# IwakuraRein/CIS-565-Final-VR-Raytracer

Measured on AMD Instinct MI355X. Metric: Mrays/s (ClosestHit+AnyHit ray queries per second) of the 1080p ReSTIR DI+GI+denoise frame; ms_per_step = ms/frame, higher is better.
Workload: dtype f32

## Files before the change

### cis-565-final-vr-raytracer_amd/csrc/dev_scene.h

```cpp
#pragma once
#include <hip/hip_runtime.h>
#include "bvh8.h"
#include "../../include/rt_abi.h"

namespace rt {

struct DevInstance {
  float o2w[12];
  float w2o[12];
  uint32_t primMesh;
  uint32_t flags;
  uint32_t pad[2];
};

struct DevTexture {
  const uint8_t* bgra;
  int32_t w, h, wrapS, wrapT, filter, pad;
};

struct DevScene {
  const Node8* nodes;
  const Tri48* tris;
  const TriRef* triRef;
  const AlphaRec* alphaRec;
  const AlphaRec* alphaByTri;
  const DevInstance* instances;
  const rt_prim_mesh* primMeshes;
  const rt_vertex* vertices;
  const uint32_t* indices;
  const rt_material* materials;
  const DevTexture* textures;
  const rt_punc_light* puncLights;
  const rt_trig_light* trigLights;
  const float* env;
  const rt_impt_samp* envAccel;
  rt_light_buf_info lightInfo;
  int32_t envW, envH;
  uint32_t numTris, numNodes;
  const struct SkyPre* sky;
  int32_t stackEntries;
  int32_t coopLive;
  float triPad;
  int32_t stackTotal;
  uint2* stackOvf; uint2* stackOvfInd;
  uint32_t stackOvfThreads;
  int32_t gangMax;
};

struct SurfRec {
  rt_vec3 position, normal, ffnormal, emission;
  float roughness, metallic;
  uint32_t matID, seed;
};

struct DevFrame {
  uint4* thisG; const uint4* lastG;
  short2* motion;
  rt_direct_reservoir* thisDirectResv; const rt_direct_reservoir* lastDirectResv;
  rt_indirect_reservoir* thisIndirectResv; const rt_indirect_reservoir* lastIndirectResv;
  uint32_t* thisLightId; const uint32_t* lastLightId;
  float4* thisDirectResult; float4* thisIndirectResult;
  float4* denoiseDirA; float4* denoiseDirB; float4* denoiseIndA; float4* denoiseIndB;
  unsigned long long* counters;
  SurfRec* surf; uint32_t* status; uint32_t* qcount; uint32_t* waveProf;
  float4* geomN; float4* geomP; float4* geomNh; float4* geomPh;
  rt_direct_reservoir* tempDirectResv;
  double* postRowSums; float* postMean;
  float4* postMipD; float4* postMipI;
  uint32_t* tileOrder;
  int32_t W, H;
  int32_t histRow0, histRow1;
  uint32_t* histMiss;
  int32_t stackLds;
  int32_t pad4;
  const uint32_t* seedIn; uint32_t* seedOut;
};

struct OmCamera {
  rt_mat4 lastProjView;
  rt_vec3 lastPosition; float pad;
};
struct DevObjMotion {
  uint32_t* instImage;
  const OmCamera* cams;
  uint32_t numInst, pad;
};

}
```

### cis-565-final-vr-raytracer_amd/csrc/rt_api.cpp

```cpp
#include <hip/hip_runtime.h>
#include <array>
#include <atomic>
#include <memory>
#include <mutex>
#include <cmath>
#include <cstdio>
#include <map>
#include <cstdlib>
#include <chrono>
#include <cstring>
#include <string>
#include <thread>
#include <unordered_map>
#include <vector>
#include "../../include/rt_abi.h"
#include "../../include/rt_cpus.h"
#include "bvh8_builder.h"
#include "stages.h"
#include "reference.h"
#include "svgf.h"
#include "gi_spatial.h"
#include "taa.h"
#include "refit.h"
#include "accel_build.h"
// ... 663 lines not shown
    if(!alphaOf.empty() && alphaOf[T.globalId]) { T.alphaIdx = alphaOf[T.globalId]; memcpy(T.omm, ommOf[T.alphaIdx].data(), sizeof(T.omm)); continue; }
    const TriRef ref = bo.triRef[T.globalId];
    const rt_prim_mesh& pm = c->primMeshes[c->instances[ref.inst].primMesh];
    const rt_material& m = c->materials[size_t(pm.materialIndex > 0 ? pm.materialIndex : 0)];
    const uint32_t* ix = &c->indices[pm.firstIndex + 3 * ref.prim];
    AlphaRec a{};
    int32_t tex = -1;
    const rt_vec2 t0 = c->vertices[pm.vertexOffset + ix[0]].texcoord, t1 = c->vertices[pm.vertexOffset + ix[1]].texcoord, t2 = c->vertices[pm.vertexOffset + ix[2]].texcoord;
    a.uv0x = t0.x; a.uv0y = t0.y; a.uv1x = t1.x; a.uv1y = t1.y; a.uv2x = t2.x; a.uv2y = t2.y;
    a.baseAlpha = m.pbrBaseColorFactor.w; a.cutoff = m.alphaCutoff; a.alphaMode = m.alphaMode;
    if(m.pbrBaseColorTexture > -1 && size_t(m.pbrBaseColorTexture) < c->devTextures.size()) {
      const DevTexture& t = c->devTextures[size_t(m.pbrBaseColorTexture)];
      tex = m.pbrBaseColorTexture; a.w = t.w; a.h = t.h; a.wrapS = t.wrapS; a.wrapT = t.wrapT; a.filter = t.filter;
    }
    T.alphaIdx = uint32_t(alpha.size());
    alpha.push_back(a); alphaTex.push_back(tex);
    std::array<uint32_t, 12> key{};
    memcpy(key.data(), &a.uv0x, 8 * sizeof(float));
    key[8] = uint32_t(m.pbrBaseColorTexture); key[9] = uint32_t(a.alphaMode); key[10] = uint32_t(a.wrapS) ^ (uint32_t(a.wrapT) << 16); key[11] = uint32_t(a.filter);
    auto it = ommCache.find(key);
    if(it == ommCache.end()) {
      std::array<uint32_t, 4> o{};
      const std::vector<uint8_t>* al = (tex >= 0 && size_t(tex) < c->hostAlpha.size()) ? &c->hostAlpha[size_t(m.pbrBaseColorTexture)] : nullptr;
      buildOpacityMap(a, al, o.data());
      it = ommCache.emplace(key, o).first;
    }
    memcpy(T.omm, it->second.data(), sizeof(T.omm));
    if(!alphaOf.empty()) { alphaOf[T.globalId] = T.alphaIdx; ommOf.resize(alpha.size()); ommOf[T.alphaIdx] = it->second; }
  }
  lt.lap("alpha records + micro-maps");
  return RT_OK;
}

int rt_build_accel(rt_ctx* c)
{
  if(!c) return RT_ERR_INVALID_ARG;
  if(!c->haveScene) return fail(c, RT_ERR_NO_SCENE, "rt_build_accel: no scene uploaded");
  RT_HIP(c, hipSetDevice(c->device));
  RT_HIP(c, syncAll(c));
  { const int rc = syncHostVertices(c); if(rc) return rc; }
  freePool(c->accelAllocs); freePool(c->rebuildAllocs);
  c->refit = rt_ctx::Refit{};
  c->rebuild = rt_ctx::Rebuild{};
  c->haveAccel = false;
  c->refN = 0;
  c->svgfValid = false;
  c->taaValid = false;
  std::shared_ptr<const HostAccel> ha;
  LoadTimer lt;
  {
    std::lock_guard<std::mutex> one(g_accelMutex);
    uint64_t k0, k1;
    sceneKey(c, k0, k1);
    lt.lap("scene key");
    if(g_accelCache && g_accelCache->key0 == k0 && g_accelCache->key1 == k1) ha = g_accelCache;
    else {
      auto fresh = std::make_shared<HostAccel>();
      fresh->key0 = k0; fresh->key1 = k1;
      const int rc = buildHostAccel(c, *fresh);
      if(rc) return rc;
      ha = fresh; g_accelCache = ha;
    }
  }
  lt.lap("host products (build or cache)");
  const BuildOutput& bo = ha->bo;
  int rc;
  {
    std::vector<AlphaRec> alpha = ha->alpha;
    for(size_t i = 0; i < alpha.size(); i++) if(ha->alphaTex[i] >= 0) alpha[i].bgra = c->devTextures[size_t(ha->alphaTex[i])].bgra;
    if((rc = upload(c, c->accelAllocs, alpha.data(), alpha.size(), &c->ds.alphaRec))) return rc;
    std::vector<AlphaRec> byTri(bo.tris.size(), AlphaRec{});
    for(size_t i = 0; i < bo.tris.size(); i++) if(!(bo.tris[i].flags & TRI_OPAQUE)) byTri[i] = alpha[bo.tris[i].alphaIdx];
    if((rc = upload(c, c->accelAllocs, byTri.data(), byTri.size(), &c->ds.alphaByTri))) return rc;
  }
  if((rc = upload(c, c->accelAllocs, bo.nodes.data(), bo.nodes.size(), &c->ds.nodes))) return rc;
  if((rc = upload(c, c->accelAllocs, bo.tris.data(), bo.tris.size(), &c->ds.tris))) return rc;
  if((rc = upload(c, c->accelAllocs, bo.triRef.data(), bo.triRef.size(), &c->ds.triRef))) return rc;
  if((rc = upload(c, c->accelAllocs, bo.instances.data(), bo.instances.size(), &c->ds.instances))) return rc;
  c->ds.numNodes = uint32_t(bo.nodes.size()); c->ds.numTris = uint32_t(bo.tris.size());
  c->ds.stackTotal = std::max(8, ((bo.maxDepth + 1 + 3) / 4) * 4);
  c->ds.stackEntries = c->ds.stackTotal;
  c->ds.triPad = bo.pad;
  { const char* e = getenv("RESTIR_COOP"); c->ds.coopLive = e ? std::max(0, std::min(64, atoi(e))) : 4; }
  { const char* e = getenv("RESTIR_GANG"); c->ds.gangMax = e ? std::max(0, std::min(7, atoi(e))) : 4; }
  c->numNodes = bo.nodes.size(); c->numTris = bo.triRef.size(); c->maxDepth = bo.maxDepth;
  c->numRefs = bo.tris.size(); c->spatialSplits = size_t(bo.spatialSplits); c->sahNodeSteps = bo.sahNodeSteps; c->sahTriSteps = bo.sahTriSteps;
  RT_HIP(c, hipDeviceSynchronize());
  lt.lap("uploads (tree, alpha records)");
  c->haveAccel = true;
  reopenPriorityDecision(c);
  if((rc = resetSeedPlane(c))) return rc;
  return ensureStackOverflow(c);
}

int rt_resize(rt_ctx* c, int w, int h)
{
  if(!c) return RT_ERR_INVALID_ARG;
  if(w <= 0 || h <= 0 || w > 32767 || h > 32767) return fail(c, RT_ERR_INVALID_ARG, "rt_resize: size must be in 1..32767 (RG16_SINT motion vectors)");
  RT_HIP(c, hipSetDevice(c->device));
  RT_HIP(c, syncAll(c));
  reopenPriorityDecision(c);
  for(void*& p : c->indA) { if(p && p != c->bufs[RT_BUF_DENOISE_IND_A]) (void)hipFree(p); p = nullptr; }
  for(int i = 0; i < RT_BUF_COUNT; i++) { if(c->bufs[i]) (void)hipFree(c->bufs[i]); c->bufs[i] = nullptr; c->bufBytes[i] = 0; }
  for(void** p : {&c->spareG, &c->spareMotion, &c->spareG2, &c->spareMotion2, &c->spareDirRes}) if(*p) { (void)hipFree(*p); *p = nullptr; }
  c->W = c->H = 0;
  for(void* p : {static_cast<void*>(c->refAcc), static_cast<void*>(c->refMean)}) if(p) (void)hipFree(p);
  c->refAcc = nullptr; c->refMean = nullptr; c->refN = 0;
  freeSvgfHistory(c);
  freeGiSpatial(c);
  freeTaaHistory(c);
  freeObjectMotion(c);
  const size_t n = size_t(w) * h, nh = size_t(w / 2) * (h / 2);
  for(int i = 0; i < RT_BUF_COUNT; i++) {
    const size_t bytes = (halfRes(i) ? nh : n) * elemBytes(i);
    const size_t alloc = bytes + (halfRes(i) ? size_t(w / 2) * (RT_PAD_ROWS / 2) : size_t(w) * RT_PAD_ROWS) * elemBytes(i) + 16;
    RT_HIP(c, hipMalloc(&c->bufs[i], alloc));
    RT_HIP(c, hipMemset(c->bufs[i], (i == RT_BUF_LIGHT_ID0 || i == RT_BUF_LIGHT_ID1) ? 0xff : 0, alloc));
    c->bufBytes[i] = bytes; c->bufAlloc[i] = alloc;
    if(i == RT_BUF_DENOISE_IND_A) {
      c->indA[0] = c->bufs[i];
      RT_HIP(c, hipMalloc(&c->indA[1], alloc));
      RT_HIP(c, hipMemset(c->indA[1], 0, alloc));
    }
    if(i == RT_BUF_GBUFFER0 || i == RT_BUF_MOTION) {
      for(void** spare : {(i == RT_BUF_MOTION) ? &c->spareMotion : &c->spareG, (i == RT_BUF_MOTION) ? &c->spareMotion2 : &c->spareG2}) {
        RT_HIP(c, hipMalloc(spare, alloc));
        RT_HIP(c, hipMemset(*spare, 0, alloc));
      }
    }
    if(i == RT_BUF_DIRECT_RESULT0) {
      RT_HIP(c, hipMalloc(&c->spareDirRes, alloc));
      RT_HIP(c, hipMemset(c->spareDirRes, 0, alloc));
    }
  }
  freePool(c->scratchAllocs);
  c->scratch = DevFrame{};
  auto alloc = [&](size_t bytes, void** out) -> int {
    RT_HIP(c, hipMalloc(out, std::max<size_t>(bytes, 256)));
    c->scratchAllocs.push_back(*out);
    RT_HIP(c, hipMemset(*out, 0, std::max<size_t>(bytes, 256)));
    return RT_OK;
  };
  DevFrame& X = c->scratch;
  int rc;
#define RT_SCRATCH(field, count, T) if((rc = alloc(size_t(count) * sizeof(T), reinterpret_cast<void**>(&X.field)))) return rc
  RT_SCRATCH(surf, n, SurfRec); RT_SCRATCH(status, n, uint32_t); RT_SCRATCH(qcount, 256, uint32_t);
  RT_SCRATCH(geomN, n, float4); RT_SCRATCH(geomP, n, float4); RT_SCRATCH(geomNh, nh, float4); RT_SCRATCH(geomPh, nh, float4);
  RT_SCRATCH(postRowSums, size_t(h) * 6, double); RT_SCRATCH(postMean, 8, float);
  RT_SCRATCH(postMipD, n + 64, float4); RT_SCRATCH(postMipI, n + 64, float4);
  RT_SCRATCH(tileOrder, (size_t(w / 2 + 7) / 8) * (size_t(h / 2 + 7) / 8 + 16 * 2) + 64 + 4096, uint32_t);
  RT_SCRATCH(seedOut, n, uint32_t); X.seedIn = X.seedOut;
#if RT_WAVEPROF
  RT_SCRATCH(waveProf, WAVEPROF_RECORDS * 16, uint32_t);
#endif
#undef RT_SCRATCH
  RT_HIP(c, hipDeviceSynchronize());
  c->W = w; c->H = h;
  if((rc = resetSeedPlane(c))) return rc;
  if(c->objMotion != RT_OBJECT_MOTION_OFF && (rc = allocObjectMotion(c))) return rc;
  return ensureStackOverflow(c);
}

static int ensureStackOverflow(rt_ctx* c)
{
  freePool(c->ovfAllocs);
  c->ds.stackOvf = c->ds.stackOvfInd = nullptr; c->ds.stackOvfThreads = 0;
// ... 1681 lines not shown
```

### cis-565-final-vr-raytracer_amd/csrc/traverse.h

```cpp
#pragma once
#include "dev_math.h"
#include "dev_scene.h"
#include "stages.h"

namespace rt {



struct RayHit {
  float t;
  uint32_t gid;
  float u, v;
};

#ifndef RT_WAVEPROF
#define RT_WAVEPROF 0
#endif
struct TravCounters {
  uint32_t nodes, tris, rounds, live;
#if RT_WAVEPROF
  uint32_t rN, rT, rC, cN, cT, cC, aTex, aOmm;
  uint32_t ph[8];
  uint32_t nph[4];
  uint32_t hl[8], he[8];
#endif
};

RT_DEV int floorMod(int i, int p)
{
  if((p & (p - 1)) == 0) return i & (p - 1);
  int m = i % p; if(m < 0) m += p;
  return m;
}
RT_DEV int wrapCoord(int i, int n, int mode)
{
  if(mode == RT_WRAP_CLAMP) return i < 0 ? 0 : (i >= n ? n - 1 : i);
  if(mode == RT_WRAP_MIRROR) {
    const int p = 2 * n;
    const int m = floorMod(i, p);
    return m < n ? m : p - 1 - m;
  }
  return floorMod(i, n);
}
RT_DEV bool wrapIsMask(int w, int h, int wrapS, int wrapT) { return (((w & (w - 1)) | (h & (h - 1))) == 0) && wrapS == RT_WRAP_REPEAT && wrapT == RT_WRAP_REPEAT; }
RT_DEV bool waveNone(bool c) { return __builtin_amdgcn_ballot_w64(c) == 0ull; }
RT_DEV f4 texelBGRA(const DevTexture& t, int x, int y)
{
  uint32_t p = gLoadU32(t.bgra + (size_t(y) * t.w + x) * 4);
  return mk4(unorm8ToFloat((p >> 16) & 0xffu), unorm8ToFloat((p >> 8) & 0xffu), unorm8ToFloat(p & 0xffu), unorm8ToFloat(p >> 24));
}
RT_DEV f4 sampleTexture(const DevScene& S, int id, f2 uv)
{
  const DevTexture t = S.textures[id];
  float fx = uv.x * float(t.w), fy = uv.y * float(t.h);
  const bool masks = waveNone(!wrapIsMask(t.w, t.h, t.wrapS, t.wrapT));
  if(t.filter == RT_FILTER_NEAREST) {
    const int xi = rt_ftoi(rt_floor(fx)), yi = rt_ftoi(rt_floor(fy));
    if(masks) return texelBGRA(t, xi & (t.w - 1), yi & (t.h - 1));
    return texelBGRA(t, wrapCoord(xi, t.w, t.wrapS), wrapCoord(yi, t.h, t.wrapT));
  }
  fx = fx - 0.5f; fy = fy - 0.5f;
  float x0f = rt_floor(fx), y0f = rt_floor(fy);
  float ax = fx - x0f, ay = fy - y0f;
  int x0 = rt_ftoi(x0f), y0 = rt_ftoi(y0f);
  int xa, xb, ya, yb;
  if(masks) { xa = x0 & (t.w - 1); xb = (x0 + 1) & (t.w - 1); ya = y0 & (t.h - 1); yb = (y0 + 1) & (t.h - 1); }
  else {
    xa = wrapCoord(x0, t.w, t.wrapS); xb = wrapCoord(x0 + 1, t.w, t.wrapS);
    ya = wrapCoord(y0, t.h, t.wrapT); yb = wrapCoord(y0 + 1, t.h, t.wrapT);
  }
  f4 top = mix(texelBGRA(t, xa, ya), texelBGRA(t, xb, ya), ax);
  f4 bot = mix(texelBGRA(t, xa, yb), texelBGRA(t, xb, yb), ax);
  return mix(top, bot, ay);
}
RT_DEV f4 envTexel(const DevScene& S, int x, int y)
{
  const float4 p = gLoadF4(S.env + (size_t(y) * S.envW + x) * 4);
  return mk4(p.x, p.y, p.z, p.w);
}
RT_DEV f4 sampleEnv(const DevScene& S, f2 uv)
{
  float fx = uv.x * float(S.envW) - 0.5f, fy = uv.y * float(S.envH) - 0.5f;
  float x0f = rt_floor(fx), y0f = rt_floor(fy);
  float ax = fx - x0f, ay = fy - y0f;
  int x0 = rt_ftoi(x0f), y0 = rt_ftoi(y0f);
  int xa = wrapCoord(x0, S.envW, RT_WRAP_REPEAT), xb = wrapCoord(x0 + 1, S.envW, RT_WRAP_REPEAT);
  int ya = wrapCoord(y0, S.envH, RT_WRAP_CLAMP), yb = wrapCoord(y0 + 1, S.envH, RT_WRAP_CLAMP);
  f4 top = mix(envTexel(S, xa, ya), envTexel(S, xb, ya), ax);
  f4 bot = mix(envTexel(S, xa, yb), envTexel(S, xb, yb), ax);
  return mix(top, bot, ay);
}

RT_DEV uint32_t pcgNext(uint32_t& state)
{
  uint32_t prev = state * 747796405u + 2891336453u;
  uint32_t word = ((prev >> ((prev >> 28u) + 4u)) ^ prev) * 277803737u;
  state = prev;
// ... 77 lines not shown
  if(F.kind == 1) a00 = gLoadU8(F.p00);
  else if(F.kind == 2) { a00 = gLoadU8(F.p00); a10 = gLoadU8(F.p10); a01 = gLoadU8(F.p01); a11 = gLoadU8(F.p11); }
  return alphaFinish(A, F, a00, a10, a01, a11, gid, raySeed);
}

RT_DEV bool intersectTri(const Tri48& T, f3 o, f3 d, float& t, float& u, float& v)
{
  const f3 e1 = mk3(T.e1x, T.e1y, T.e1z), e2 = mk3(T.e2x, T.e2y, T.e2z), v0 = mk3(T.v0x, T.v0y, T.v0z);
  const f3 p = cross(d, e2);
  const float det = dot(e1, p);
  if(T.flags & TRI_NOCULL) { if(det == 0.0f || rt_isnan(det)) return false; }
  else {
    const float sdet = (T.flags & TRI_FLIP) ? -det : det;
    if(!(sdet > 0.0f)) return false;
  }
  const float inv = 1.0f / det;
  const f3 tv = o - v0;
  u = dot(tv, p) * inv;
  if(!(u >= 0.0f && u <= 1.0f)) return false;
  const f3 q = cross(tv, e1);
  v = dot(d, q) * inv;
  if(!(v >= 0.0f && u + v <= 1.0f)) return false;
  t = dot(e2, q) * inv;
  return !rt_isnan(t);
}
RT_DEV float hitPointPad(f3 o, f3 d, float pad, float t)
{
  const float om = fmaxf(fmaxf(rt_abs(o.x), rt_abs(o.y)), rt_abs(o.z)), dm = fmaxf(fmaxf(rt_abs(d.x), rt_abs(d.y)), rt_abs(d.z));
  return pad + (om + t * dm) * 4.76837158203125e-07f;
}
RT_DEV bool hitInsidePaddedBox(const Tri48& T, f3 o, f3 d, float buildPad, float t)
{
  const float pad = hitPointPad(o, d, buildPad, t);
  const f3 e1 = mk3(T.e1x, T.e1y, T.e1z), e2 = mk3(T.e2x, T.e2y, T.e2z), v0 = mk3(T.v0x, T.v0y, T.v0z);
  const f3 h = o + d * t;
  const f3 lo = mk3((v0.x + fminf(fminf(0.0f, e1.x), e2.x)) - pad, (v0.y + fminf(fminf(0.0f, e1.y), e2.y)) - pad, (v0.z + fminf(fminf(0.0f, e1.z), e2.z)) - pad);
  const f3 hi = mk3((v0.x + fmaxf(fmaxf(0.0f, e1.x), e2.x)) + pad, (v0.y + fmaxf(fmaxf(0.0f, e1.y), e2.y)) + pad, (v0.z + fmaxf(fmaxf(0.0f, e1.z), e2.z)) + pad);
  return h.x >= lo.x && h.x <= hi.x && h.y >= lo.y && h.y <= hi.y && h.z >= lo.z && h.z <= hi.z;
}

RT_DEV float cvtByte(uint32_t w, int j) { return float((w >> (8 * j)) & 0xffu); }

struct Trav {
  f3 o, d;
  float idx, idy, idz;
  uint32_t octinv;
  uint2 ngroup;
  uint2 tgroup;
  int sp;
  float tmax;
  uint32_t seed;
  RayHit hit;
  uint32_t rec;
  bool found;
  bool isAny;
};

RT_DEV bool travHasTris(const Trav& T) { return T.tgroup.y != 0u; }
RT_DEV bool travHasNodes(const Trav& T) { return T.ngroup.y > 0x00FFFFFFu || T.sp > 0; }

template <int MODE>
RT_DEV bool travInit(Trav& T, f3 o, f3 d, float tmax, uint32_t raySeed)
{
  const bool ANY = MODE == 2 ? T.isAny : MODE == 1;
  T.o = o; T.d = d; T.tmax = tmax; T.seed = raySeed; T.found = false; T.sp = 0;
  T.hit.t = ANY ? tmax : RT_INFINITY;
  T.hit.gid = 0xffffffffu; T.hit.u = 0.f; T.hit.v = 0.f; T.rec = 0xffffffffu;
  T.ngroup = make_uint2(0u, 0u);
  T.tgroup = make_uint2(0u, 0u);
  if(hasNan(o) || hasNan(d) || !(T.hit.t > 0.0f)) return false;
  const float eps = 1e-20f;
  T.idx = 1.0f / (rt_abs(d.x) > eps ? d.x : (d.x < 0.0f ? -eps : eps));
  T.idy = 1.0f / (rt_abs(d.y) > eps ? d.y : (d.y < 0.0f ? -eps : eps));
  T.idz = 1.0f / (rt_abs(d.z) > eps ? d.z : (d.z < 0.0f ? -eps : eps));
  T.octinv = (((d.x < 0.0f) ? 1u : 0u) | ((d.y < 0.0f) ? 2u : 0u) | ((d.z < 0.0f) ? 4u : 0u)) ^ 7u;
  T.ngroup = make_uint2(0u, 0x80000000u);
  return true;
}

RT_DEV uint2* stackOverflowSlot(const DevScene& S, int sp)
{
  const size_t thread = size_t(blockIdx.x) * blockDim.x + threadIdx.x;
  return S.stackOvf + (thread * size_t(S.stackTotal - S.stackEntries) + size_t(sp - S.stackEntries));
}
RT_DEV uint2 stackPop(const DevScene& S, Trav& T, uint2* stack)
{
  --T.sp;
  if(__builtin_expect(T.sp < S.stackEntries, 1)) return ldsLoadU2(stack + T.sp * 64);
  return gLoadU2(stackOverflowSlot(S, T.sp));
}
RT_DEV void stackPush(const DevScene& S, Trav& T, uint2* stack, uint2 g)
{
  if(__builtin_expect(T.sp < S.stackEntries, 1)) ldsStoreU2(stack + (T.sp++) * 64, g);
  else if(T.sp < S.stackTotal) { gStoreU2(stackOverflowSlot(S, T.sp), g); T.sp++; }
}

struct NodeRegs { uint4 n0, n1, n2, n3, n4; };
RT_DEV uint32_t travNodeSelect(const DevScene& S, Trav& T, uint2* stack)
{
  uint2 ngroup = T.ngroup;
  if(ngroup.y <= 0x00FFFFFFu) ngroup = stackPop(S, T, stack);
  const uint32_t hits = ngroup.y;
  const uint32_t bit = 31u - uint32_t(__clz(int(hits)));
  ngroup.y &= ~(1u << bit);
  if(ngroup.y > 0x00FFFFFFu) stackPush(S, T, stack, ngroup);
  const uint32_t slot = (bit - 24u) ^ T.octinv;
  const uint32_t rel = uint32_t(__popc(hits & ~(0xFFFFFFFFu << slot) & 0xFFu));
  T.ngroup.y = 0u;
  return ngroup.x + rel;
}
RT_DEV NodeRegs nodeLoad(const DevScene& S, uint32_t index)
{
  const uint4* np = reinterpret_cast<const uint4*>(S.nodes + index);
  NodeRegs N; N.n0 = gLoadU4(np); N.n1 = gLoadU4(np + 1); N.n2 = gLoadU4(np + 2); N.n3 = gLoadU4(np + 3); N.n4 = gLoadU4(np + 4);
  return N;
}
RT_DEV void travNodeTest(Trav& T, const NodeRegs& N)
{
  const uint4 n0 = N.n0, n1 = N.n1, n2 = N.n2, n3 = N.n3, n4 = N.n4;
  const bool nx = T.d.x < 0.0f, ny = T.d.y < 0.0f, nz = T.d.z < 0.0f;
  const uint32_t octinv = T.octinv;
  const uint32_t octinv4 = octinv * 0x01010101u;
  const float adjx = rt_u2f((n0.w & 0xffu) << 23) * T.idx;
  const float adjy = rt_u2f(((n0.w >> 8) & 0xffu) << 23) * T.idy;
  const float adjz = rt_u2f(((n0.w >> 16) & 0xffu) << 23) * T.idz;
  const float orgx = (rt_u2f(n0.x) - T.o.x) * T.idx, orgy = (rt_u2f(n0.y) - T.o.y) * T.idy, orgz = (rt_u2f(n0.z) - T.o.z) * T.idz;
  const uint32_t imask = n0.w >> 24;
  uint32_t hitmask = 0;
#pragma unroll
  for(int half = 0; half < 2; half++) {
    const uint32_t meta4 = half ? n1.w : n1.z;
    const uint32_t isInner4 = (meta4 & (meta4 << 1)) & 0x10101010u;
    const uint32_t innerMask4 = (isInner4 >> 4) * 0xffu;
    const uint32_t bitIndex4 = (meta4 ^ (octinv4 & innerMask4)) & 0x1F1F1F1Fu;
    const uint32_t childBits4 = (meta4 >> 5) & 0x07070707u;
    const uint32_t qlx = half ? n2.y : n2.x, qly = half ? n2.w : n2.z, qlz = half ? n3.y : n3.x;
    const uint32_t qhx = half ? n3.w : n3.z, qhy = half ? n4.y : n4.x, qhz = half ? n4.w : n4.z;
    const uint32_t nearx = nx ? qhx : qlx, farx = nx ? qlx : qhx;
    const uint32_t neary = ny ? qhy : qly, fary = ny ? qly : qhy;
    const uint32_t nearz = nz ? qhz : qlz, farz = nz ? qlz : qhz;
#pragma unroll
    for(int j = 0; j < 4; j++) {
      const float tlx = __builtin_fmaf(cvtByte(nearx, j), adjx, orgx), thx = __builtin_fmaf(cvtByte(farx, j), adjx, orgx);
      const float tly = __builtin_fmaf(cvtByte(neary, j), adjy, orgy), thy = __builtin_fmaf(cvtByte(fary, j), adjy, orgy);
      const float tlz = __builtin_fmaf(cvtByte(nearz, j), adjz, orgz), thz = __builtin_fmaf(cvtByte(farz, j), adjz, orgz);
      const float tn = fmaxf(fmaxf(tlx, tly), fmaxf(tlz, 0.0f));
      const float tf = fminf(fminf(thx, thy), fminf(thz, T.hit.t));
      if(tn <= tf) hitmask |= ((childBits4 >> (8 * j)) & 0xffu) << ((bitIndex4 >> (8 * j)) & 0xffu);
    }
  }
  T.ngroup = make_uint2(n1.x, (hitmask & 0xFF000000u) | imask);
  T.tgroup = make_uint2(n1.y, hitmask & 0x00FFFFFFu);
}
RT_DEV void travNode(const DevScene& S, Trav& T, uint2* stack, TravCounters& tc)
{
  const uint32_t index = travNodeSelect(S, T, stack);
  const NodeRegs N = nodeLoad(S, index);
  tc.nodes++;
  travNodeTest(T, N);
}

struct TriRegs { uint4 a, b, c, om; };
RT_DEV TriRegs triLoad(const DevScene& S, uint32_t triIndex)
{
  const uint4* tp = reinterpret_cast<const uint4*>(S.tris + triIndex);
  TriRegs Q; Q.a = gLoadU4(tp); Q.b = gLoadU4(tp + 1); Q.c = gLoadU4(tp + 2); Q.om = gLoadU4(tp + 3);
// ... 27 lines not shown
    (void)tc;
#endif
    if(state == 1u) return 1;
    if(state == 2u) { uint32_t hs = candidateSeed(seed, R.globalId); return !(rnd(hs) > 0.0f) ? 1 : 0; }
    return 2;
  }
  return 1;
}
RT_DEV bool triCandidate(const DevScene& S, uint32_t triIndex, f3 o, f3 d, bool ANY, float tmax, float curT, uint32_t curG, uint32_t seed, float& t, float& u, float& v,
                         uint32_t& gid, TravCounters& tc)
{
  const TriRegs Q = triLoad(S, triIndex);
  uint32_t alphaIdx;
  const int s = triCandidateGeom(S, Q, o, d, ANY, tmax, curT, curG, seed, t, u, v, gid, alphaIdx, tc);
  if(s == 2) return hitTestAlpha(S, alphaIdx, gid, u, v, seed);
  return s == 1;
}

template <int MODE>
RT_DEV void travTri(const DevScene& S, Trav& T, TravCounters& tc)
{
  const bool ANY = MODE == 2 ? T.isAny : MODE == 1;
  const uint32_t bit = 31u - uint32_t(__clz(int(T.tgroup.y)));
  T.tgroup.y &= ~(1u << bit);
  tc.tris++;
  float t, u, v; uint32_t gid;
  if(!triCandidate(S, T.tgroup.x + bit, T.o, T.d, ANY, T.tmax, T.hit.t, T.hit.gid, T.seed, t, u, v, gid, tc)) return;
  T.hit.t = t; T.hit.gid = gid; T.hit.u = u; T.hit.v = v; T.rec = T.tgroup.x + bit;
  T.found = true;
  if(ANY) { T.tgroup.y = 0u; T.ngroup.y = 0u; T.sp = 0; }
}

RT_DEV float laneF(float v, int l) { return rt_u2f(uint32_t(__builtin_amdgcn_readlane(int(rt_f2u(v)), l))); }
RT_DEV uint32_t laneU(uint32_t v, int l) { return uint32_t(__builtin_amdgcn_readlane(int(v), l)); }

template <int MODE>
RT_DEV void travTriCoop(const DevScene& S, Trav& T, unsigned long long triMask, TravCounters& tc)
{
  const int lane = int(threadIdx.x) & 63;
  const unsigned long long present = __ballot(1);
  const int rank = __popcll(present & ((1ull << lane) - 1ull)), np = __popcll(present);
  while(triMask != 0ull) {
    const int l = __builtin_ctzll(triMask);
    triMask &= triMask - 1ull;
    const f3 o = mk3(laneF(T.o.x, l), laneF(T.o.y, l), laneF(T.o.z, l)), d = mk3(laneF(T.d.x, l), laneF(T.d.y, l), laneF(T.d.z, l));
    const uint32_t tbase = laneU(T.tgroup.x, l), seed = laneU(T.seed, l);
    uint32_t tbits = laneU(T.tgroup.y, l);
    const float tmax = laneF(T.tmax, l);
    const bool ANY = MODE == 2 ? (laneU(T.isAny ? 1u : 0u, l) != 0u) : MODE == 1;
    float bt = laneF(T.hit.t, l), bu = 0.0f, bv = 0.0f;
    uint32_t bg = laneU(T.hit.gid, l), br = 0u;
    bool found = false;
    if(lane == l) tc.tris += uint32_t(__popc(tbits));
    while(tbits != 0u && !(ANY && found)) {
      int mine = -1, j = 0;
      while(tbits != 0u && j < np) {
        const int k = 31 - __clz(int(tbits));
        tbits &= ~(1u << k);
        if(rank == j) mine = k;
        j++;
      }
      float t = 0.0f, u = 0.0f, v = 0.0f; uint32_t gid = 0u;
      bool ok = false;
      if(mine >= 0) ok = triCandidate(S, tbase + uint32_t(mine), o, d, ANY, tmax, bt, bg, seed, t, u, v, gid, tc);
      unsigned long long okm = __ballot(ok ? 1 : 0);
      while(okm != 0ull) {
        const int w = __builtin_ctzll(okm);
        okm &= okm - 1ull;
        const float wt = laneF(t, w); const uint32_t wg = laneU(gid, w);
        if(ANY || wt < bt || (wt == bt && wg < bg)) { bt = wt; bg = wg; bu = laneF(u, w); bv = laneF(v, w); br = tbase + laneU(uint32_t(mine), w); found = true; }
        if(ANY) break;
      }
    }
    if(lane == l) {
      T.tgroup.y = 0u;
      if(found) {
        T.hit.t = bt; T.hit.gid = bg; T.hit.u = bu; T.hit.v = bv; T.rec = br; T.found = true;
        if(ANY) { T.ngroup.y = 0u; T.sp = 0; }
      }
    }
  }
}

template <int ANY>
RT_DEV bool travRound(const DevScene& S, Trav& T, bool live, uint2* stack, TravCounters& tc)
{
  tc.rounds++; tc.live += live ? 1u : 0u;
  const bool wantTri = live && travHasTris(T);
  const bool wantNode = live && !wantTri;
  const int nT = __popcll(__ballot(wantTri ? 1 : 0)), nN = __popcll(__ballot(wantNode ? 1 : 0));
  if(nT >= nN) { if(wantTri) travTri<ANY>(S, T, tc); }
  else { if(wantNode) travNode(S, T, stack, tc); }
  return live && (travHasTris(T) || travHasNodes(T));
}

template <int ANY>
RT_DEV bool travRoundMasked(const DevScene& S, Trav& T, bool live, unsigned long long liveMask, uint2* stack, TravCounters& tc)
{
  tc.rounds++; tc.live += live ? 1u : 0u;
  const bool wantTri = live && travHasTris(T);
  const unsigned long long triMask = __ballot(wantTri ? 1 : 0);
  const int nLive = __popcll(liveMask), nT = __popcll(triMask), nN = nLive - nT;
#if RT_WAVEPROF
  const uint64_t c0 = clock64();
#endif
  if(nLive <= S.coopLive) {
    if(nT > 0) travTriCoop<ANY>(S, T, triMask, tc);
    if(live && travHasNodes(T)) travNode(S, T, stack, tc);
  } else if(nT >= nN) { if(wantTri) travTri<ANY>(S, T, tc); }
  else { if(live && !wantTri) travNode(S, T, stack, tc); }
#if RT_WAVEPROF
  {
    const uint32_t dc = uint32_t(clock64() - c0);
    if(nLive <= S.coopLive) { tc.rC++; tc.cC += dc; } else if(nT >= nN) { tc.rT++; tc.cT += dc; } else { tc.rN++; tc.cN += dc; }
    const int ex = nLive <= S.coopLive ? nLive : (nT >= nN ? nT : nN);
    tc.hl[(nLive - 1) >> 3]++; tc.he[(max(ex, 1) - 1) >> 3]++;
  }
#endif
  return live && (travHasTris(T) || travHasNodes(T));
}

template <int ANY>
RT_DEV bool traceRay(const DevScene& S, f3 o, f3 d, float tmax, uint32_t raySeed, uint2* stack, RayHit& hit, TravCounters& tc)
{
  Trav T;
  bool live = travInit<ANY>(T, o, d, tmax, raySeed);
  unsigned long long liveMask = __ballot(live ? 1 : 0);
  while(liveMask != 0ull) {
    live = travRoundMasked<ANY>(S, T, live, liveMask, stack, tc);
    liveMask = __ballot(live ? 1 : 0);
  }
  hit = T.hit;
  return T.found;
}

RT_DEV bool traceRaySeeded(const DevScene& S, f3 o, f3 d, uint32_t raySeed, uint32_t seedTri, uint2* stack, RayHit& hit, uint32_t& rec, TravCounters& tc)
{
  float st = 0.0f, su = 0.0f, sv = 0.0f; uint32_t sg = 0xffffffffu;
  bool seeded = false;
  if(seedTri < S.numTris) {
    tc.tris++;
    seeded = triCandidate(S, seedTri, o, d, false, RT_INFINITY, RT_INFINITY, 0xffffffffu, raySeed, st, su, sv, sg, tc);
  }
  Trav T;
  bool live = travInit<0>(T, o, d, RT_INFINITY, raySeed);
  if(live && seeded) { T.hit.t = st; T.hit.gid = sg; T.hit.u = su; T.hit.v = sv; T.rec = seedTri; T.found = true; }
  unsigned long long liveMask = __ballot(live ? 1 : 0);
  while(liveMask != 0ull) {
    live = travRoundMasked<0>(S, T, live, liveMask, stack, tc);
    liveMask = __ballot(live ? 1 : 0);
  }
  hit = T.hit; rec = T.rec;
  return T.found;
}

constexpr int POOL_SLOT_F4 = 2;
constexpr int POOL_BYTES = 128 * 32 + 128;

RT_DEV void poolPut(float4* pool, int slot, f3 o, f3 d, float tmax, uint32_t seed)
{
  pool[slot * POOL_SLOT_F4] = make_float4(o.x, o.y, o.z, d.x);
  pool[slot * POOL_SLOT_F4 + 1] = make_float4(d.y, d.z, tmax, rt_u2f(seed));
}
RT_DEV RayHit poolGet(const float4* pool, int slot)
{
  const float4 r = pool[slot * POOL_SLOT_F4];
  RayHit h; h.t = r.x; h.gid = rt_f2u(r.y); h.u = r.z; h.v = r.w;
  return h;
}
RT_DEV void poolPutRec(float4* pool, int slot, uint32_t rec) { reinterpret_cast<uint32_t*>(pool + slot * POOL_SLOT_F4 + 1)[0] = rec; }
RT_DEV uint32_t poolGetRec(const float4* pool, int slot) { return reinterpret_cast<const uint32_t*>(pool + slot * POOL_SLOT_F4 + 1)[0]; }
RT_DEV void waveLdsSync() { __builtin_amdgcn_fence(__ATOMIC_SEQ_CST, "wavefront"); __builtin_amdgcn_wave_barrier(); }

RT_DEV void tracePool(const DevScene& S, float4* pool, bool hasC, bool hasS, uint2* stack, TravCounters& tc)
{
  unsigned char* list = reinterpret_cast<unsigned char*>(pool + 128 * POOL_SLOT_F4);
  const int lane = int(threadIdx.x) & 63;
  const unsigned long long lt = (1ull << lane) - 1ull;
  const unsigned long long mC = __ballot(hasC ? 1 : 0), mS = __ballot(hasS ? 1 : 0);
  const int nC = __popcll(mC), n = nC + __popcll(mS);
  if(n == 0) return;
  if(hasC) list[__popcll(mC & lt)] = (unsigned char)(lane * 2);
  if(hasS) list[nC + __popcll(mS & lt)] = (unsigned char)(lane * 2 + 1);
  waveLdsSync();
  int next = 0, mySlot = 0;
  bool live = false;
  Trav T;
  for(;;) {
    unsigned long long liveMask = __ballot(live ? 1 : 0);
    const unsigned long long idle = ~liveMask;
    if(next < n && idle != 0ull) {
      const int item = next + __popcll(idle & lt);
      if(!live && item < n) {
        mySlot = int(list[item]);
        const float4 a = pool[mySlot * POOL_SLOT_F4], b = pool[mySlot * POOL_SLOT_F4 + 1];
        T.isAny = (mySlot & 1) != 0;
        live = travInit<2>(T, mk3(a.x, a.y, a.z), mk3(a.w, b.x, b.y), b.z, rt_f2u(b.w));
        if(!live) pool[mySlot * POOL_SLOT_F4] = make_float4(T.hit.t, rt_u2f(T.hit.gid), T.hit.u, T.hit.v);
      }
      next = min(n, next + __popcll(idle));
      liveMask = __ballot(live ? 1 : 0);
    }
    if(liveMask == 0ull) {
      if(next >= n) break;
      continue;
    }
    const bool still = travRoundMasked<2>(S, T, live, liveMask, stack, tc);
    if(live && !still) pool[mySlot * POOL_SLOT_F4] = make_float4(T.hit.t, rt_u2f(T.hit.gid), T.hit.u, T.hit.v);
    live = still;
  }
  waveLdsSync();
}

template <int K, bool ANY>
RT_DEV void tracePoolTiles(const DevScene& S, float4* pool, uint32_t have , uint2* stack, TravCounters& tc)
{
  unsigned char* list = reinterpret_cast<unsigned char*>(pool + K * 64 * POOL_SLOT_F4);
  const int lane = int(threadIdx.x) & 63;
  const unsigned long long lt = (1ull << lane) - 1ull;
  int n = 0;
#pragma unroll
  for(int k = 0; k < K; k++) {
    const bool h = (have >> k) & 1u;
    const unsigned long long m = __ballot(h ? 1 : 0);
    if(h) list[n + __popcll(m & lt)] = (unsigned char)(k * 64 + lane);
    n += __popcll(m);
  }
  if(n == 0) return;
  waveLdsSync();
  int next = 0, mySlot = 0;
  bool live = false;
  Trav T;
  for(;;) {
    unsigned long long liveMask = __ballot(live ? 1 : 0);
    const unsigned long long idle = ~liveMask;
    if(next < n && idle != 0ull) {
      const int item = next + __popcll(idle & lt);
      if(!live && item < n) {
        mySlot = int(list[item]);
        const float4 a = pool[mySlot * POOL_SLOT_F4], b = pool[mySlot * POOL_SLOT_F4 + 1];
        live = travInit<ANY>(T, mk3(a.x, a.y, a.z), mk3(a.w, b.x, b.y), b.z, rt_f2u(b.w));
        if(!live) pool[mySlot * POOL_SLOT_F4] = make_float4(T.hit.t, rt_u2f(T.hit.gid), T.hit.u, T.hit.v);
      }
      next = min(n, next + __popcll(idle));
      liveMask = __ballot(live ? 1 : 0);
    }
    if(liveMask == 0ull) {
      if(next >= n) break;
      continue;
    }
    const bool still = travRoundMasked<ANY>(S, T, live, liveMask, stack, tc);
    if(live && !still) pool[mySlot * POOL_SLOT_F4] = make_float4(T.hit.t, rt_u2f(T.hit.gid), T.hit.u, T.hit.v);
    live = still;
  }
  waveLdsSync();
}

#ifndef RT_LAT
#define RT_LAT 0
#endif
#if RT_LAT
constexpr int WIDE_G = 8;
constexpr int WIDE_RAYS = 64 / WIDE_G;
#define RT_DPP_XOR1 0xB1
#define RT_DPP_XOR2 0x4E
#define RT_DPP_HALF_MIRROR 0x141
template <int CTRL> RT_DEV uint32_t dppU(uint32_t v) { return uint32_t(__builtin_amdgcn_update_dpp(0, int(v), CTRL, 0xf, 0xf, true)); }
template <int CTRL> RT_DEV float dppF(float v) { return rt_u2f(dppU<CTRL>(rt_f2u(v))); }
RT_DEV uint32_t groupOr(uint32_t v)
{
  v |= dppU<RT_DPP_XOR1>(v);
  v |= dppU<RT_DPP_XOR2>(v);
  v |= dppU<RT_DPP_HALF_MIRROR>(v);
  return v;
}
struct WideCand { float t; uint32_t gid; float u, v; uint32_t rec; };
template <int CTRL> RT_DEV void candMinStep(WideCand& c)
{
  const float ot = dppF<CTRL>(c.t); const uint32_t og = dppU<CTRL>(c.gid); const float ou = dppF<CTRL>(c.u), ov = dppF<CTRL>(c.v); const uint32_t orc = dppU<CTRL>(c.rec);
  const bool take = ot < c.t || (ot == c.t && og < c.gid);
  c.t = take ? ot : c.t; c.gid = take ? og : c.gid; c.u = take ? ou : c.u; c.v = take ? ov : c.v; c.rec = take ? orc : c.rec;
}
RT_DEV void groupMinCand(WideCand& c) { candMinStep<RT_DPP_XOR1>(c); candMinStep<RT_DPP_XOR2>(c); candMinStep<RT_DPP_HALF_MIRROR>(c); }

RT_DEV uint2 stackPopW(Trav& T, const uint2* stack) { --T.sp; return ldsLoadU2(stack + T.sp * WIDE_RAYS); }
RT_DEV void stackPushW(Trav& T, uint2* stack, uint2 g, int j) { if(j == 0) ldsStoreU2(stack + T.sp * WIDE_RAYS, g); T.sp++; }
RT_DEV uint32_t travNodeSelectW(Trav& T, uint2* stack, int j)
{
  uint2 ngroup = T.ngroup;
  if(ngroup.y <= 0x00FFFFFFu) ngroup = stackPopW(T, stack);
  const uint32_t hits = ngroup.y;
  const uint32_t bit = 31u - uint32_t(__clz(int(hits)));
  ngroup.y &= ~(1u << bit);
  if(ngroup.y > 0x00FFFFFFu) stackPushW(T, stack, ngroup, j);
  const uint32_t slot = (bit - 24u) ^ T.octinv;
  const uint32_t rel = uint32_t(__popc(hits & ~(0xFFFFFFFFu << slot) & 0xFFu));
  T.ngroup.y = 0u;
  return ngroup.x + rel;
}
RT_DEV uint32_t byteOf(uint32_t lo, uint32_t hi, int j) { return ((j < 4 ? lo : hi) >> (8 * (j & 3))) & 0xffu; }
RT_DEV void travNodeTestW(Trav& T, const NodeRegs& N, int j)
{
  const uint4 n0 = N.n0, n1 = N.n1, n2 = N.n2, n3 = N.n3, n4 = N.n4;
  const bool nx = T.d.x < 0.0f, ny = T.d.y < 0.0f, nz = T.d.z < 0.0f;
  const float adjx = rt_u2f((n0.w & 0xffu) << 23) * T.idx;
  const float adjy = rt_u2f(((n0.w >> 8) & 0xffu) << 23) * T.idy;
  const float adjz = rt_u2f(((n0.w >> 16) & 0xffu) << 23) * T.idz;
  const float orgx = (rt_u2f(n0.x) - T.o.x) * T.idx, orgy = (rt_u2f(n0.y) - T.o.y) * T.idy, orgz = (rt_u2f(n0.z) - T.o.z) * T.idz;
  const uint32_t imask = n0.w >> 24;
  const uint32_t meta = byteOf(n1.z, n1.w, j);
  const uint32_t isInner = (meta & (meta << 1)) & 0x10u;
  const uint32_t bitIndex = (meta ^ (isInner ? T.octinv : 0u)) & 0x1Fu;
  const uint32_t childBits = (meta >> 5) & 0x07u;
  const float qlx = float(byteOf(n2.x, n2.y, j)), qly = float(byteOf(n2.z, n2.w, j)), qlz = float(byteOf(n3.x, n3.y, j));
  const float qhx = float(byteOf(n3.z, n3.w, j)), qhy = float(byteOf(n4.x, n4.y, j)), qhz = float(byteOf(n4.z, n4.w, j));
  const float tlx = __builtin_fmaf(nx ? qhx : qlx, adjx, orgx), thx = __builtin_fmaf(nx ? qlx : qhx, adjx, orgx);
  const float tly = __builtin_fmaf(ny ? qhy : qly, adjy, orgy), thy = __builtin_fmaf(ny ? qly : qhy, adjy, orgy);
  const float tlz = __builtin_fmaf(nz ? qhz : qlz, adjz, orgz), thz = __builtin_fmaf(nz ? qlz : qhz, adjz, orgz);
  const float tn = fmaxf(fmaxf(tlx, tly), fmaxf(tlz, 0.0f));
  const float tf = fminf(fminf(thx, thy), fminf(thz, T.hit.t));
  const uint32_t hitmask = groupOr((tn <= tf) ? (childBits << bitIndex) : 0u);
  T.ngroup = make_uint2(n1.x, (hitmask & 0xFF000000u) | imask);
  T.tgroup = make_uint2(n1.y, hitmask & 0x00FFFFFFu);
}
template <int MODE>
RT_DEV void travTriW(const DevScene& S, Trav& T, int j, TravCounters& tc)
{
  const bool ANY = MODE == 2 ? T.isAny : MODE == 1;
  uint32_t rem = T.tgroup.y;
  int mine = -1;
#pragma unroll
  for(int k = 0; k < WIDE_G; k++) {
    if(rem != 0u) {
      const int b = 31 - __clz(int(rem));
      if(k == j) mine = b;
      rem &= ~(1u << b);
    }
  }
  T.tgroup.y = rem;
  WideCand c; c.t = __builtin_huge_valf(); c.gid = 0xffffffffu; c.u = 0.0f; c.v = 0.0f; c.rec = 0xffffffffu;
  bool ok = false;
#if RT_WAVEPROF
#define RT_PH(k) { __builtin_amdgcn_s_waitcnt(0); const uint64_t pn = clock64(); tc.ph[k] += uint32_t(pn - pc); pc = pn; }
  uint64_t pc = clock64(); tc.ph[7]++;
#else
#define RT_PH(k)
#endif
  if(mine >= 0) {
    float t, u, v; uint32_t gid, alphaIdx;
    const uint32_t ti = T.tgroup.x + uint32_t(mine);
    const TriRegs Q = triLoad(S, ti);
    const uint4* ap = reinterpret_cast<const uint4*>(S.alphaByTri + ti);
    AlphaRegs A; A.r0 = gLoadU4(ap); A.r1 = gLoadU4(ap + 1); A.r2 = gLoadU4(ap + 2); A.r3 = gLoadU4(ap + 3);
    RT_PH(0)
    const int s = triCandidateGeom(S, Q, T.o, T.d, ANY, T.tmax, T.hit.t, T.hit.gid, T.seed, t, u, v, gid, alphaIdx, tc);
    ok = s == 1;
    RT_PH(1)
    if(s == 2) {
      const AlphaFetch Fh = alphaAddr(A, u, v, reinterpret_cast<const uint8_t*>(S.alphaRec));
      RT_PH(2)
      uint8_t a00 = 0, a10 = 0, a01 = 0, a11 = 0;
      if(Fh.kind == 1) a00 = gLoadU8(Fh.p00);
      else if(Fh.kind == 2) { a00 = gLoadU8(Fh.p00); a10 = gLoadU8(Fh.p10); a01 = gLoadU8(Fh.p01); a11 = gLoadU8(Fh.p11); }
      RT_PH(3)
      ok = alphaFinish(A, Fh, a00, a10, a01, a11, gid, T.seed);
      RT_PH(4)
    }
    if(ok) { c.t = t; c.gid = gid; c.u = u; c.v = v; c.rec = ti; }
  }
  RT_PH(5)
  groupMinCand(c);
  const bool any = c.t < __builtin_huge_valf();
  if(any && (ANY || c.t < T.hit.t || (c.t == T.hit.t && c.gid < T.hit.gid))) {
    T.hit.t = c.t; T.hit.gid = c.gid; T.hit.u = c.u; T.hit.v = c.v; T.rec = c.rec;
    T.found = true;
    if(ANY) { T.tgroup.y = 0u; T.ngroup.y = 0u; T.sp = 0; }
  }
  RT_PH(6)
#undef RT_PH
  (void)ok;
}
template <int MODE>
RT_DEV bool travRoundW(const DevScene& S, Trav& T, bool live, int j, uint2* stack, TravCounters& tc)
{
  bool wantTri = live && travHasTris(T);
  bool wantNode = live && !wantTri;
  {
    const int nT = __popcll(__ballot(wantTri ? 1 : 0)), nN = __popcll(__ballot(wantNode ? 1 : 0));
    if(nT >= nN) wantNode = false; else wantTri = false;
  }
  if(wantTri) travTriW<MODE>(S, T, j, tc);
#if RT_WAVEPROF
  if(wantNode) {
    __builtin_amdgcn_s_waitcnt(0); const uint64_t q0 = clock64();
    const uint32_t ni = travNodeSelectW(T, stack, j);
    __builtin_amdgcn_s_waitcnt(0); const uint64_t q1 = clock64();
    const NodeRegs N = nodeLoad(S, ni);
    __builtin_amdgcn_s_waitcnt(0); const uint64_t q2 = clock64();
    travNodeTestW(T, N, j);
    const uint64_t q3 = clock64();
    tc.nph[0] += uint32_t(q1 - q0); tc.nph[1] += uint32_t(q2 - q1); tc.nph[2] += uint32_t(q3 - q2); tc.nph[3]++;
  }
#else
  if(wantNode) { const NodeRegs N = nodeLoad(S, travNodeSelectW(T, stack, j)); travNodeTestW(T, N, j); }
#endif
  return live && (travHasTris(T) || travHasNodes(T));
}

constexpr int GANG_BOX_UINT2 = 20;
constexpr int GANG_SCAN = 2;
constexpr int GANG_EXTRA = 20;
RT_DEV uint32_t leaderBits(unsigned long long m) { return uint32_t(((m & 0x0101010101010101ull) * 0x0102040810204080ull) >> 56); }
RT_DEV int nthSetBitFromTop(uint32_t v, int n)
{
  for(int k = 0; k < n; k++) v &= ~(1u << (31 - __clz(int(v))));
  return 31 - __clz(int(v));
}
RT_DEV uint32_t dropTopBits(uint32_t v, int n) { for(int k = 0; k < n; k++) v &= ~(1u << (31 - __clz(int(v)))); return v; }

template <bool REC>
RT_DEV void gangTail(const DevScene& S, float4* pool, uint2* waveStack, Trav& T, bool& live, int mySlot, TravCounters& tc)
{
  const int lane = int(threadIdx.x) & 63, j = lane & (WIDE_G - 1), g = lane >> 3;
  float4* gbox = reinterpret_cast<float4*>(waveStack + size_t(S.stackEntries) * WIDE_RAYS);
  uint32_t* rbox = reinterpret_cast<uint32_t*>(gbox + WIDE_RAYS);
  const int wideRoom = S.stackEntries - S.stackTotal;
  bool working = false;
  int og = g;
  uint32_t wm = 0u;
  uint32_t lastOwners = 0u;
  for(;;) {
    const uint32_t owners = leaderBits(__ballot(live ? 1 : 0));
    if(owners == 0u) break;
    if(owners != lastOwners) {
      lastOwners = owners;
      const int n = __popc(owners);
      const bool mine = (owners >> g) & 1u;
      const uint32_t freeM = leaderBits(__ballot((!working && !mine) ? 1 : 0));
      const bool adopt = !working && !mine;
      if(mine && !working) {
        if(T.ngroup.y > 0x00FFFFFFu) { if(__builtin_expect(T.sp >= S.stackEntries, 0)) __builtin_trap(); stackPushW(T, waveStack + g, T.ngroup, j); T.ngroup.y = 0u; }
        og = g;
      }
      if(adopt) {
        uint32_t o = owners;
        for(int k = __popc(freeM & ((1u << g) - 1u)) % n; k > 0; k--) o &= o - 1u;
        og = __ffs(int(o)) - 1;
      }
      waveLdsSync();
      const int src = og * WIDE_G;
      const int slot = __shfl(mySlot, src);
      const int sp = __shfl(T.sp, src);
      const float bt = __shfl(T.hit.t, src), bu = __shfl(T.hit.u, src), bv = __shfl(T.hit.v, src);
      const uint32_t bg = uint32_t(__shfl(int(T.hit.gid), src));
      const int any = __shfl(T.isAny ? 1 : 0, src);
      const uint32_t brc = REC ? uint32_t(__shfl(int(T.rec), src)) : 0xffffffffu;
      if(adopt) {
        const float4 a = pool[slot * POOL_SLOT_F4], b = pool[slot * POOL_SLOT_F4 + 1];
        T.isAny = any != 0;
        (void)travInit<2>(T, mk3(a.x, a.y, a.z), mk3(a.w, b.x, b.y), b.z, rt_f2u(b.w));
        T.ngroup.y = 0u; T.tgroup.y = 0u;
        T.sp = sp; T.hit.t = bt; T.hit.gid = bg; T.hit.u = bu; T.hit.v = bv; T.rec = brc;
      }
      working = true;
// ... 130 lines not shown
```

Before: 1494.

## Finish straggler rays with 8-lane-per-ray wide traversal in persistent loops

Once the ray queue is drained and a wave has at most wideTail live rays (default 8), those rays are redistributed so that each is traversed cooperatively by 8 lanes, using the wide node/triangle test path. Ray state is gathered from the owning lane with ds_bpermute, the owner's LDS and overflow stack is reused via a lane-offset pointer, and results are permuted back at the end. The aim is to cut the long tail of low-occupancy rounds in which a few rays keep a whole wave busy. In exchange it adds permute overhead and more code and register pressure, and it only applies when the full wave is active.

```diff
diff --git a/cis-565-final-vr-raytracer_amd/csrc/dev_scene.h b/cis-565-final-vr-raytracer_amd/csrc/dev_scene.h
--- a/cis-565-final-vr-raytracer_amd/csrc/dev_scene.h
+++ b/cis-565-final-vr-raytracer_amd/csrc/dev_scene.h
@@ -44,6 +44,7 @@
   int32_t stackTotal;
   uint2* stackOvf; uint2* stackOvfInd;
   uint32_t stackOvfThreads;
+  int32_t wideTail;
   int32_t gangMax;
 };
 
diff --git a/cis-565-final-vr-raytracer_amd/csrc/rt_api.cpp b/cis-565-final-vr-raytracer_amd/csrc/rt_api.cpp
--- a/cis-565-final-vr-raytracer_amd/csrc/rt_api.cpp
+++ b/cis-565-final-vr-raytracer_amd/csrc/rt_api.cpp
@@ -769,6 +769,7 @@
   c->ds.stackEntries = c->ds.stackTotal;
   c->ds.triPad = bo.pad;
   { const char* e = getenv("RESTIR_COOP"); c->ds.coopLive = e ? std::max(0, std::min(64, atoi(e))) : 4; }
+  { const char* e = getenv("RESTIR_WIDE_TAIL"); c->ds.wideTail = e ? std::max(0, std::min(8, atoi(e))) : 8; }
   { const char* e = getenv("RESTIR_GANG"); c->ds.gangMax = e ? std::max(0, std::min(7, atoi(e))) : 4; }
   c->numNodes = bo.nodes.size(); c->numTris = bo.triRef.size(); c->maxDepth = bo.maxDepth;
   c->numRefs = bo.tris.size(); c->spatialSplits = size_t(bo.spatialSplits); c->sahNodeSteps = bo.sahNodeSteps; c->sahTriSteps = bo.sahTriSteps;
diff --git a/cis-565-final-vr-raytracer_amd/csrc/traverse.h b/cis-565-final-vr-raytracer_amd/csrc/traverse.h
--- a/cis-565-final-vr-raytracer_amd/csrc/traverse.h
+++ b/cis-565-final-vr-raytracer_amd/csrc/traverse.h
@@ -13,6 +13,9 @@
   float u, v;
 };
 
+#ifndef RT_LAT
+#define RT_LAT 0
+#endif
 #ifndef RT_WAVEPROF
 #define RT_WAVEPROF 0
 #endif
@@ -256,6 +259,12 @@
 {
   const size_t thread = size_t(blockIdx.x) * blockDim.x + threadIdx.x;
   return S.stackOvf + (thread * size_t(S.stackTotal - S.stackEntries) + size_t(sp - S.stackEntries));
+}
+RT_DEV uint2* splitLdsPointer(uint2* p)
+{
+  uint32_t a = uint32_t(uintptr_t((RT_AS_LDS uint2*)p));
+  asm volatile("" : "+v"(a));
+  return (uint2*)((RT_AS_LDS uint2*)uintptr_t(a));
 }
 RT_DEV uint2 stackPop(const DevScene& S, Trav& T, uint2* stack)
 {
@@ -449,6 +458,9 @@
   }
 }
 
+template <int MODE> RT_DEV void wideTail(const DevScene& S, Trav& T, bool live, unsigned long long liveMask, uint2* stack, TravCounters& tc);
+RT_DEV int tailThreshold(const DevScene& S) { return (!RT_LAT && __ballot(1) == ~0ull) ? S.wideTail : 0; }
+
 template <int ANY>
 RT_DEV bool travRound(const DevScene& S, Trav& T, bool live, uint2* stack, TravCounters& tc)
 {
@@ -553,6 +565,8 @@
   int next = 0, mySlot = 0;
   bool live = false;
   Trav T;
+  const int tailAt = tailThreshold(S);
+  stack = splitLdsPointer(stack);
   for(;;) {
     unsigned long long liveMask = __ballot(live ? 1 : 0);
     const unsigned long long idle = ~liveMask;
@@ -572,6 +586,11 @@
       if(next >= n) break;
       continue;
     }
+    if(next >= n && __popcll(liveMask) <= tailAt) {
+      wideTail<2>(S, T, live, liveMask, stack, tc);
+      if(live) pool[mySlot * POOL_SLOT_F4] = make_float4(T.hit.t, rt_u2f(T.hit.gid), T.hit.u, T.hit.v);
+      break;
+    }
     const bool still = travRoundMasked<2>(S, T, live, liveMask, stack, tc);
     if(live && !still) pool[mySlot * POOL_SLOT_F4] = make_float4(T.hit.t, rt_u2f(T.hit.gid), T.hit.u, T.hit.v);
     live = still;
@@ -598,6 +617,7 @@
   int next = 0, mySlot = 0;
   bool live = false;
   Trav T;
+  const int tailAt = tailThreshold(S);
   for(;;) {
     unsigned long long liveMask = __ballot(live ? 1 : 0);
     const unsigned long long idle = ~liveMask;
@@ -616,6 +636,11 @@
       if(next >= n) break;
       continue;
     }
+    if(next >= n && __popcll(liveMask) <= tailAt) {
+      wideTail<ANY>(S, T, live, liveMask, stack, tc);
+      if(live) pool[mySlot * POOL_SLOT_F4] = make_float4(T.hit.t, rt_u2f(T.hit.gid), T.hit.u, T.hit.v);
+      break;
+    }
     const bool still = travRoundMasked<ANY>(S, T, live, liveMask, stack, tc);
     if(live && !still) pool[mySlot * POOL_SLOT_F4] = make_float4(T.hit.t, rt_u2f(T.hit.gid), T.hit.u, T.hit.v);
     live = still;
@@ -623,10 +648,6 @@
   waveLdsSync();
 }
 
-#ifndef RT_LAT
-#define RT_LAT 0
-#endif
-#if RT_LAT
 constexpr int WIDE_G = 8;
 constexpr int WIDE_RAYS = 64 / WIDE_G;
 #define RT_DPP_XOR1 0xB1
@@ -650,6 +671,7 @@
 }
 RT_DEV void groupMinCand(WideCand& c) { candMinStep<RT_DPP_XOR1>(c); candMinStep<RT_DPP_XOR2>(c); candMinStep<RT_DPP_HALF_MIRROR>(c); }
 
+#if RT_LAT
 RT_DEV uint2 stackPopW(Trav& T, const uint2* stack) { --T.sp; return ldsLoadU2(stack + T.sp * WIDE_RAYS); }
 RT_DEV void stackPushW(Trav& T, uint2* stack, uint2 g, int j) { if(j == 0) ldsStoreU2(stack + T.sp * WIDE_RAYS, g); T.sp++; }
 RT_DEV uint32_t travNodeSelectW(Trav& T, uint2* stack, int j)
@@ -665,6 +687,7 @@
   T.ngroup.y = 0u;
   return ngroup.x + rel;
 }
+#endif
 RT_DEV uint32_t byteOf(uint32_t lo, uint32_t hi, int j) { return ((j < 4 ? lo : hi) >> (8 * (j & 3))) & 0xffu; }
 RT_DEV void travNodeTestW(Trav& T, const NodeRegs& N, int j)
 {
@@ -690,10 +713,11 @@
   T.ngroup = make_uint2(n1.x, (hitmask & 0xFF000000u) | imask);
   T.tgroup = make_uint2(n1.y, hitmask & 0x00FFFFFFu);
 }
-template <int MODE>
+template <int MODE, bool TAIL = false>
 RT_DEV void travTriW(const DevScene& S, Trav& T, int j, TravCounters& tc)
 {
   const bool ANY = MODE == 2 ? T.isAny : MODE == 1;
+  const float tmax = TAIL ? T.hit.t : T.tmax;
   uint32_t rem = T.tgroup.y;
   int mine = -1;
 #pragma unroll
@@ -714,13 +738,14 @@
 #define RT_PH(k)
 #endif
   if(mine >= 0) {
+    if(TAIL) tc.tris++;
     float t, u, v; uint32_t gid, alphaIdx;
     const uint32_t ti = T.tgroup.x + uint32_t(mine);
     const TriRegs Q = triLoad(S, ti);
     const uint4* ap = reinterpret_cast<const uint4*>(S.alphaByTri + ti);
     AlphaRegs A; A.r0 = gLoadU4(ap); A.r1 = gLoadU4(ap + 1); A.r2 = gLoadU4(ap + 2); A.r3 = gLoadU4(ap + 3);
     RT_PH(0)
-    const int s = triCandidateGeom(S, Q, T.o, T.d, ANY, T.tmax, T.hit.t, T.hit.gid, T.seed, t, u, v, gid, alphaIdx, tc);
+    const int s = triCandidateGeom(S, Q, T.o, T.d, ANY, tmax, T.hit.t, T.hit.gid, T.seed, t, u, v, gid, alphaIdx, tc);
     ok = s == 1;
     RT_PH(1)
     if(s == 2) {
@@ -747,6 +772,101 @@
 #undef RT_PH
   (void)ok;
 }
+
+RT_DEV uint32_t bpermU(int srcLane, uint32_t v) { return uint32_t(__builtin_amdgcn_ds_bpermute(srcLane << 2, int(v))); }
+RT_DEV float bpermF(int srcLane, float v) { return rt_u2f(bpermU(srcLane, rt_f2u(v))); }
+struct OwnerStack { uint2* col; int delta; };
+RT_DEV uint2* ownerOverflowSlot(const DevScene& S, const OwnerStack& K, int sp)
+{
+  const size_t thread = size_t(blockIdx.x) * blockDim.x + size_t(int(threadIdx.x) + K.delta);
+  return S.stackOvf + (thread * size_t(S.stackTotal - S.stackEntries) + size_t(sp - S.stackEntries));
+}
+RT_DEV uint2 stackPopO(const DevScene& S, Trav& T, const OwnerStack& K)
+{
+  --T.sp;
+  if(__builtin_expect(T.sp < S.stackEntries, 1)) return ldsLoadU2(K.col + T.sp * 64);
+  __builtin_amdgcn_fence(__ATOMIC_ACQUIRE, "wavefront");
+  return gLoadU2(ownerOverflowSlot(S, K, T.sp));
+}
+RT_DEV void stackPushO(const DevScene& S, Trav& T, const OwnerStack& K, uint2 g, int j)
+{
+  if(__builtin_expect(T.sp < S.stackEntries, 1)) { if(j == 0) ldsStoreU2(K.col + T.sp * 64, g); T.sp++; }
+  else if(T.sp < S.stackTotal) { if(j == 0) gStoreU2(ownerOverflowSlot(S, K, T.sp), g); __builtin_amdgcn_fence(__ATOMIC_RELEASE, "wavefront"); T.sp++; }
+}
+RT_DEV uint32_t travNodeSelectO(const DevScene& S, Trav& T, const OwnerStack& K, int j)
+{
+  uint2 ngroup = T.ngroup;
+  if(ngroup.y <= 0x00FFFFFFu) ngroup = stackPopO(S, T, K);
+  const uint32_t hits = ngroup.y;
+  const uint32_t bit = 31u - uint32_t(__clz(int(hits)));
+  ngroup.y &= ~(1u << bit);
+  if(ngroup.y > 0x00FFFFFFu) stackPushO(S, T, K, ngroup, j);
+  const uint32_t slot = (bit - 24u) ^ T.octinv;
+  const uint32_t rel = uint32_t(__popc(hits & ~(0xFFFFFFFFu << slot) & 0xFFu));
+  T.ngroup.y = 0u;
+  return ngroup.x + rel;
+}
+template <int MODE>
+RT_DEV void wideTail(const DevScene& S, Trav& T, bool live, unsigned long long liveMask, uint2* stack, TravCounters& tc)
+{
+  const int lane = int(threadIdx.x) & 63, j = lane & (WIDE_G - 1), g = lane >> 3;
+  int owner = lane;
+  bool wl = false;
+  {
+    unsigned long long m = liveMask;
+#pragma unroll
+    for(int k = 0; k < WIDE_RAYS; k++) {
+      if(m != 0ull) { if(g == k) { owner = __builtin_ctzll(m); wl = true; } m &= m - 1ull; }
+    }
+  }
+  Trav W;
+  W.o = mk3(bpermF(owner, T.o.x), bpermF(owner, T.o.y), bpermF(owner, T.o.z));
+  W.d = mk3(bpermF(owner, T.d.x), bpermF(owner, T.d.y), bpermF(owner, T.d.z));
+  W.idx = bpermF(owner, T.idx); W.idy = bpermF(owner, T.idy); W.idz = bpermF(owner, T.idz);
+  W.octinv = bpermU(owner, T.octinv);
+  W.ngroup = make_uint2(bpermU(owner, T.ngroup.x), bpermU(owner, T.ngroup.y));
+  W.tgroup = make_uint2(bpermU(owner, T.tgroup.x), bpermU(owner, T.tgroup.y));
+  W.sp = int(bpermU(owner, uint32_t(T.sp)));
+  W.tmax = 0.0f;
+  W.seed = bpermU(owner, T.seed);
+  W.hit.t = bpermF(owner, T.hit.t); W.hit.gid = bpermU(owner, T.hit.gid); W.hit.u = bpermF(owner, T.hit.u); W.hit.v = bpermF(owner, T.hit.v);
+  W.rec = bpermU(owner, T.rec);
+  W.isAny = MODE == 2 ? (bpermU(owner, T.isAny ? 1u : 0u) != 0u) : false;
+  W.found = false;
+  OwnerStack K;
+  K.delta = owner - lane;
+  K.col = stack + K.delta;
+  unsigned long long wm = __ballot(wl ? 1 : 0);
+  while(wm != 0ull) {
+    if(j == 0) { tc.rounds++; tc.live += wl ? 1u : 0u; }
+    bool wantTri = wl && travHasTris(W);
+    bool wantNode = wl && !wantTri;
+    {
+      const int nT = __popcll(__ballot(wantTri ? 1 : 0)), nN = __popcll(wm) - nT;
+      if(nT >= nN) wantNode = false; else wantTri = false;
+    }
+#if RT_WAVEPROF
+    const uint64_t c0 = clock64();
+    const int ex = __popcll(__ballot((wantTri || wantNode) ? 1 : 0));
+#endif
+    if(wantTri) travTriW<MODE, true>(S, W, j, tc);
+    if(wantNode) {
+      if(j == 0) tc.nodes++;
+      const NodeRegs N = nodeLoad(S, travNodeSelectO(S, W, K, j));
+      travNodeTestW(W, N, j);
+    }
+#if RT_WAVEPROF
+    { tc.rC++; tc.cC += uint32_t(clock64() - c0); tc.hl[(__popcll(wm) / WIDE_G - 1) >> 3]++; tc.he[(max(ex, 1) - 1) >> 3]++; }
+#endif
+    wl = wl && (travHasTris(W) || travHasNodes(W));
+    wm = __ballot(wl ? 1 : 0);
+  }
+  const int src = live ? __popcll(liveMask & ((1ull << lane) - 1ull)) * WIDE_G : lane;
+  const float ht = bpermF(src, W.hit.t), hu = bpermF(src, W.hit.u), hv = bpermF(src, W.hit.v);
+  const uint32_t hg = bpermU(src, W.hit.gid), hr = bpermU(src, W.rec), hf = bpermU(src, W.found ? 1u : 0u);
+  if(live) { T.hit.t = ht; T.hit.gid = hg; T.hit.u = hu; T.hit.v = hv; T.rec = hr; T.found = T.found || hf != 0u; }
+}
+#if RT_LAT
 template <int MODE>
 RT_DEV bool travRoundW(const DevScene& S, Trav& T, bool live, int j, uint2* stack, TravCounters& tc)
 {
```

Measured after the change: 1520, median of 6. 1.02x the previous value.
